# JonasFrey96/Visual-Odom-Pipeline

Hardware: NVIDIA B200
Metric: tracked_keypoints_per_sec (higher is better)
Workload: dtype u8

## Files before the change

visual-odom-pipeline_b200/csrc/klt_capi.cu:

```cuda
#include <chrono>
#include <cmath>
#include <cstdio>
#include <cstdlib>
#include <cstring>
#include <algorithm>
#include <atomic>
#include <condition_variable>
#include <thread>
#include <immintrin.h>
#include <functional>
#include <mutex>
#include <new>
#include <vector>

#include "klt_common.cuh"

using namespace klt;

struct klt_ctx {
    int device = 0;
    int sm_count = 0;
    int cc_major = 0, cc_minor = 0;
    char name[128] = {0};
    cudaStream_t stream = nullptr;
// ... 52 lines not shown
    if (guard__.err != cudaSuccess) return (klt_status)guard__.err

klt_status ensure_device_ws(klt_ctx* ctx, size_t bytes)
{
    if (bytes <= ctx->d_ws_bytes) return KLT_OK;
    ctx->reuse_key[0] = 0;
    if (ctx->d_ws) { KLT_CUDA(cudaStreamSynchronize(ctx->stream)); KLT_CUDA(cudaStreamSynchronize(ctx->stream2)); cudaFree(ctx->d_ws); ctx->d_ws = nullptr; ctx->d_ws_bytes = 0; }
    bytes = align_up(bytes + bytes / 4, 1 << 20);
    cudaError_t e = cudaMalloc(&ctx->d_ws, bytes);
    if (e != cudaSuccess) return e == cudaErrorMemoryAllocation ? KLT_ERR_OUT_OF_MEMORY : (klt_status)e;
    if (cudaMemset(ctx->d_ws, 0, bytes) != cudaSuccess || cudaDeviceSynchronize() != cudaSuccess) cudaGetLastError();
    ctx->d_ws_bytes = bytes;
    return KLT_OK;
}

klt_status ensure_host_ws(klt_ctx* ctx, size_t bytes)
{
    if (bytes <= ctx->h_ws_bytes) return KLT_OK;
    if (ctx->h_ws) { KLT_CUDA(cudaStreamSynchronize(ctx->stream)); KLT_CUDA(cudaStreamSynchronize(ctx->stream2)); cudaFreeHost(ctx->h_ws); ctx->h_ws = nullptr; ctx->h_ws_dev = nullptr; ctx->h_ws_bytes = 0; }
    bytes = align_up(bytes + bytes / 4, 1 << 16);
    cudaError_t e = cudaHostAlloc(&ctx->h_ws, bytes, cudaHostAllocMapped);
    if (e != cudaSuccess) return e == cudaErrorMemoryAllocation ? KLT_ERR_OUT_OF_MEMORY : (klt_status)e;
    void* alias = nullptr;
    ctx->h_ws_dev = (cudaHostGetDevicePointer(&alias, ctx->h_ws, 0) == cudaSuccess) ? static_cast<uint8_t*>(alias) : nullptr;
    cudaGetLastError();
    ctx->h_ws_bytes = bytes;
    return KLT_OK;
}

}

struct klt_ctx::Stager {
    static constexpr int kHelpers = 3;
    static constexpr int kParts = kHelpers + 1;
    std::thread threads[kHelpers];
    std::mutex m;
    std::condition_variable cv;
    std::atomic<unsigned> gen{0};
    std::atomic<int> done[2];
    bool stop = false;
    const uint8_t* src[2] = {nullptr, nullptr};
    uint8_t* dst[2] = {nullptr, nullptr};
    size_t bytes[2] = {0, 0};

    static void slice(size_t total, int part, size_t& off, size_t& len)
    {
        const size_t per = ((total + kParts - 1) / kParts + 63) & ~(size_t)63;
        off = std::min(total, per * (size_t)part);
        len = std::min(total - off, per);
    }
    void copy_part(int job, int part)
    {
        size_t off, len;
        slice(bytes[job], part, off, len);
        if (len) std::memcpy(dst[job] + off, src[job] + off, len);
    }
    void worker(int part)
    {
        unsigned seen = 0;
        for (;;) {
            bool got = false;
            const auto t0 = std::chrono::steady_clock::now();
            for (int spin = 0;; ++spin) {
                if (gen.load(std::memory_order_acquire) != seen) { got = true; break; }
                _mm_pause();
                if ((spin & 255) == 255 && std::chrono::steady_clock::now() - t0 > std::chrono::microseconds(200)) break;
            }
            if (!got) {
                std::unique_lock<std::mutex> lk(m);
                cv.wait(lk, [&] { return stop || gen.load(std::memory_order_acquire) != seen; });
                if (stop) return;
            }
            seen = gen.load(std::memory_order_acquire);
            if (seen == 0xffffffffu) return;
            copy_part(0, part);
            done[0].fetch_add(1, std::memory_order_release);
            copy_part(1, part);
            done[1].fetch_add(1, std::memory_order_release);
        }
    }
    bool start()
    {
        done[0].store(0); done[1].store(0);
        try {
            for (int i = 0; i < kHelpers; ++i) threads[i] = std::thread(&Stager::worker, this, i);
        } catch (...) {
            shutdown();
            return false;
        }
        return true;
    }
    void shutdown()
    {
        { std::lock_guard<std::mutex> lk(m); stop = true; gen.store(0xffffffffu, std::memory_order_release); }
        cv.notify_all();
        for (auto& t : threads) if (t.joinable()) t.join();
    }
    void post(const uint8_t* s0, uint8_t* d0, size_t b0, const uint8_t* s1, uint8_t* d1, size_t b1)
    {
        src[0] = s0; dst[0] = d0; bytes[0] = b0; src[1] = s1; dst[1] = d1; bytes[1] = b1;
        done[0].store(0, std::memory_order_relaxed); done[1].store(0, std::memory_order_relaxed);
        {
            std::lock_guard<std::mutex> lk(m);
            unsigned g = gen.load(std::memory_order_relaxed) + 1;
            if (g == 0 || g == 0xffffffffu) g = 1;
            gen.store(g, std::memory_order_release);
        }
        cv.notify_all();
    }
    void finish_job(int job)
    {
        copy_part(job, kHelpers);
        while (done[job].load(std::memory_order_acquire) < kHelpers) _mm_pause();
    }
};

namespace {

bool is_pageable(const void* p)
{
    struct Entry { uintptr_t page; bool pageable; };
    thread_local Entry cache[64] = {};
    const uintptr_t page = reinterpret_cast<uintptr_t>(p) >> 12;
    Entry& e = cache[(page ^ (page >> 6)) & 63];
    if (e.page == page && page != 0) return e.pageable;
    cudaPointerAttributes a;
    const cudaError_t err = cudaPointerGetAttributes(&a, p);
    bool pageable = true;
    if (err != cudaSuccess) cudaGetLastError();
    else pageable = (a.type == cudaMemoryTypeUnregistered);
    e.page = page; e.pageable = pageable;
    return pageable;
}

klt_status ensure_host_in(klt_ctx* ctx, size_t bytes)
{
    if (bytes <= ctx->h_in_bytes) return KLT_OK;
    if (ctx->h_in) {
        KLT_CUDA(cudaStreamSynchronize(ctx->stream));
        KLT_CUDA(cudaStreamSynchronize(ctx->stream2));
        cudaFreeHost(ctx->h_in); ctx->h_in = nullptr; ctx->h_in_bytes = 0;
    }
    bytes = align_up(bytes + bytes / 4, 1 << 16);
    cudaError_t e = cudaHostAlloc(&ctx->h_in, bytes, cudaHostAllocDefault);
    if (e != cudaSuccess) return e == cudaErrorMemoryAllocation ? KLT_ERR_OUT_OF_MEMORY : (klt_status)e;
    ctx->h_in_bytes = bytes;
    return KLT_OK;
}

}

namespace {

struct PyrReuse { const unsigned* hash_new; const unsigned* hash_old; unsigned* hash_clear; unsigned long long* skipped; unsigned mask; };

klt_status pyr_build_one_launch(klt_ctx* ctx, const uint8_t* d_img, const klt_pyr_layout* lay, uint8_t* d_pyr, int first_item,
                                int n_items, cudaStream_t stream, const PyrReuse* reuse = nullptr)
{
    const int n_steps = lay->top;
    const uint8_t* src[KLT_MAX_LEVELS];
    uint8_t* dst[KLT_MAX_LEVELS];
    int w[KLT_MAX_LEVELS], h[KLT_MAX_LEVELS];
    long long sp[KLT_MAX_LEVELS], sb[KLT_MAX_LEVELS], dp[KLT_MAX_LEVELS], db[KLT_MAX_LEVELS];
    for (int l = 0; l < n_steps; ++l) {
        const klt_level& a = lay->level[l];
        const klt_level& b = lay->level[l + 1];
        src[l] = ((l == 0) ? d_img : d_pyr + a.offset) + (int64_t)first_item * a.batch_stride;
        dst[l] = d_pyr + b.offset + (int64_t)first_item * b.batch_stride;
        w[l] = a.w; h[l] = a.h; sp[l] = a.pitch; sb[l] = a.batch_stride; dp[l] = b.pitch; db[l] = b.batch_stride;
    }
    PyrFused P;
    long long n_cnt = 0;
    klt_status s = pyr_fused_plan(P, n_steps, src, dst, w, h, sp, sb, dp, db, n_items, ctx->sm_count, &n_cnt);
    if (s != KLT_OK) return s;
    cudaStreamCaptureStatus cap = cudaStreamCaptureStatusNone;
    if (cudaStreamIsCapturing(stream, &cap) != cudaSuccess) { cudaGetLastError(); cap = cudaStreamCaptureStatusNone; }
    const bool device_gen = cap != cudaStreamCaptureStatusNone;
    const long long key[6] = {lay->level[0].w, lay->level[0].h, n_steps, n_items, lay->level[0].pitch, P.s[0].rows};
    std::lock_guard<std::mutex> guard(ctx->lk_mutex);
    klt_ctx::PyrScratch* slot = nullptr;
    for (auto& sc : ctx->pyr_scratch)
        if (sc.stream == stream && std::memcmp(sc.key, key, sizeof(key)) == 0) { slot = &sc; break; }
    const size_t words = ((size_t)(n_cnt > 0 ? n_cnt : 0) + 1) / 2 * 2 + 2;
    if (!slot) {
        if (device_gen) return KLT_ERR_UNSUPPORTED;
        if (ctx->pyr_scratch.size() >= 64) {
            KLT_CUDA(cudaDeviceSynchronize());
            for (auto& sc : ctx->pyr_scratch) cudaFree(sc.cnt);
            ctx->pyr_scratch.clear();
        }
        klt_ctx::PyrScratch fresh = {stream, nullptr, nullptr, n_cnt, 0u, {key[0], key[1], key[2], key[3], key[4], key[5]}};
        void* p = nullptr;
        cudaError_t e = cudaMalloc(&p, 2 * words * sizeof(unsigned));
        if (e != cudaSuccess) return e == cudaErrorMemoryAllocation ? KLT_ERR_OUT_OF_MEMORY : (klt_status)e;
        e = cudaMemset(p, 0, 2 * words * sizeof(unsigned));
        if (e == cudaSuccess) e = cudaDeviceSynchronize();
        if (e != cudaSuccess) { cudaFree(p); return (klt_status)e; }
        fresh.cnt = static_cast<unsigned*>(p);
        fresh.cnt_dev = fresh.cnt + words;
        try { ctx->pyr_scratch.push_back(fresh); } catch (const std::bad_alloc&) { cudaFree(p); return KLT_ERR_OUT_OF_MEMORY; }
        slot = &ctx->pyr_scratch.back();
    }
    if (device_gen) {
        P.cnt = slot->cnt_dev;
        P.gen = 0u;
        P.done = reinterpret_cast<unsigned long long*>(slot->cnt_dev + words - 2);
    } else {
        P.cnt = slot->cnt;
        P.gen = ++slot->gen;
        P.done = nullptr;
    }
    if (reuse) { P.hash_new = reuse->hash_new; P.hash_old = reuse->hash_old; P.hash_clear = reuse->hash_clear; P.skipped = reuse->skipped; P.reuse_mask = reuse->mask; }
    s = pyr_fused_launch(P, device_gen, stream);
    if (s != KLT_OK && !device_gen) --slot->gen;
    return s;
}

void make_view(const klt_pyr_layout* lay, const uint8_t* img, const uint8_t* pyr, int first_item, int item_stride, PyrView& v)
{
    v.top = lay->top;
    for (int l = 0; l <= lay->top; ++l) {
        const klt_level& s = lay->level[l];
        v.lv[l].data = ((l == 0) ? img : pyr + s.offset) + (int64_t)first_item * s.batch_stride;
        v.lv[l].batch_stride = s.batch_stride * item_stride;
        v.lv[l].pitch = (int)s.pitch;
        v.lv[l].w = s.w;
        v.lv[l].h = s.h;
        v.lv[l].aligned4 = (((uintptr_t)v.lv[l].data | (uintptr_t)s.pitch | (uintptr_t)s.batch_stride) & 3) == 0;
    }
}

klt_status check_layout(const klt_pyr_layout* lay)
{
    if (!lay || lay->top < 0 || lay->top >= KLT_MAX_LEVELS || lay->batch <= 0) return KLT_ERR_INVALID_ARG;
    for (int l = 0; l <= lay->top; ++l) {
        const klt_level& s = lay->level[l];
        if (s.w <= 0 || s.h <= 0 || s.pitch < s.w || s.pitch > 0x7fffffffLL) return KLT_ERR_INVALID_ARG;
        if (lay->batch > 1 && s.batch_stride < s.pitch * (int64_t)(s.h - 1) + s.w) return KLT_ERR_INVALID_ARG;
    }
    return KLT_OK;
}

void normalise_criteria(const klt_lk_params* p, int& max_count, double& eps2)
{
    double eps;
    if ((p->crit_type & KLT_TERM_COUNT) == 0) max_count = 30;
    else max_count = p->crit_max_count < 0 ? 0 : (p->crit_max_count > 100 ? 100 : p->crit_max_count);
    if ((p->crit_type & KLT_TERM_EPS) == 0) eps = 0.01;
    else eps = p->crit_eps < 0. ? 0. : (p->crit_eps > 10. ? 10. : p->crit_eps);
    eps2 = eps * eps;
}

void set_eps_brackets(LKLaunch& L)
{
    if (L.eps2 >= 1e-30 && L.eps2 <= 1e30) {
        L.eps2_lo = std::nextafterf((float)(L.eps2 * (1.0 - 1.0 / 1048576.0)), -1.f);
        L.eps2_hi = std::nextafterf((float)(L.eps2 * (1.0 + 1.0 / 1048576.0)), 3.0e38f);
    } else {
        L.eps2_lo = -1.f;
        L.eps2_hi = __builtin_inff();
    }
}

}

extern "C" {

int klt_version(void) { return KLT_B200_VERSION; }

const char* klt_status_string(klt_status s)
{
    switch (s) {
        case KLT_OK: return "ok";
        case KLT_ERR_INVALID_ARG: return "invalid argument (cv2 would raise an assertion error)";
        case KLT_ERR_UNSUPPORTED: return "valid for OpenCV but outside libklt_b200 limits";
        case KLT_ERR_NO_DEVICE: return "no sm_100 CUDA device available (there is no CPU fallback)";
        case KLT_ERR_OUT_OF_MEMORY: return "out of memory";
        case KLT_ERR_INTERNAL: return "internal error";
        default: return s > 0 ? cudaGetErrorString((cudaError_t)s) : "unknown status";
    }
}

klt_status klt_create(int device, klt_ctx** out)
{
    if (!out) return KLT_ERR_INVALID_ARG;
    *out = nullptr;
    int n = 0;
    if (cudaGetDeviceCount(&n) != cudaSuccess || n <= 0 || device < 0 || device >= n) {
        cudaGetLastError();
        return KLT_ERR_NO_DEVICE;
    }
    cudaDeviceProp prop;
    KLT_CUDA(cudaGetDeviceProperties(&prop, device));
    if (prop.major != 10) return KLT_ERR_NO_DEVICE;
    DeviceGuard guard(device);
    if (guard.err != cudaSuccess) return (klt_status)guard.err;
    klt_ctx* ctx = new (std::nothrow) klt_ctx();
    if (!ctx) return KLT_ERR_OUT_OF_MEMORY;
    ctx->device = device;
    ctx->sm_count = prop.multiProcessorCount;
    ctx->cc_major = prop.major;
    ctx->cc_minor = prop.minor;
    std::snprintf(ctx->name, sizeof(ctx->name), "%s", prop.name);
    cudaError_t e = cudaStreamCreateWithFlags(&ctx->stream, cudaStreamNonBlocking);
    if (e == cudaSuccess) e = cudaStreamCreateWithFlags(&ctx->stream2, cudaStreamNonBlocking);
    if (e == cudaSuccess) e = cudaEventCreateWithFlags(&ctx->ev2, cudaEventDisableTiming);
    if (e != cudaSuccess) {
        if (ctx->stream) cudaStreamDestroy(ctx->stream);
        if (ctx->stream2) cudaStreamDestroy(ctx->stream2);
        delete ctx;
        return (klt_status)e;
    }
    klt_status s = lk_init(device);
    if (s != KLT_OK) { cudaStreamDestroy(ctx->stream); cudaStreamDestroy(ctx->stream2); cudaEventDestroy(ctx->ev2); delete ctx; return s; }
    *out = ctx;
    return KLT_OK;
}

klt_status klt_destroy(klt_ctx* ctx)
{
    if (!ctx) return KLT_OK;
    DeviceGuard guard(ctx->device);
    if (ctx->stream) { cudaStreamSynchronize(ctx->stream); cudaStreamDestroy(ctx->stream); }
    if (ctx->stream2) { cudaStreamSynchronize(ctx->stream2); cudaStreamDestroy(ctx->stream2); }
    if (ctx->ev2) cudaEventDestroy(ctx->ev2);
    if (ctx->stager) { ctx->stager->shutdown(); delete ctx->stager; ctx->stager = nullptr; }
    if (ctx->d_ws) cudaFree(ctx->d_ws);
    if (ctx->h_ws) cudaFreeHost(ctx->h_ws);
    if (ctx->h_in) cudaFreeHost(ctx->h_in);
    if (ctx->d_hash) cudaFree(ctx->d_hash);
    cudaDeviceSynchronize();
    for (auto& sc : ctx->pyr_scratch) cudaFree(sc.cnt);
    for (auto& t : ctx->bilateral_tabs) cudaFree(t.d_tab);
    delete ctx;
    return KLT_OK;
}

klt_status klt_device_info(klt_ctx* ctx, int* sm_count, int* cc_major, int* cc_minor, char* name, int name_len)
{
    if (!ctx) return KLT_ERR_INVALID_ARG;
    if (sm_count) *sm_count = ctx->sm_count;
    if (cc_major) *cc_major = ctx->cc_major;
    if (cc_minor) *cc_minor = ctx->cc_minor;
    if (name && name_len > 0) std::snprintf(name, (size_t)name_len, "%s", ctx->name);
    return KLT_OK;
}

klt_status klt_host_alloc(void** ptr, int64_t bytes)
{
    if (!ptr || bytes <= 0) return KLT_ERR_INVALID_ARG;
    cudaError_t e = cudaMallocHost(ptr, (size_t)bytes);
    if (e != cudaSuccess) { *ptr = nullptr; return e == cudaErrorMemoryAllocation ? KLT_ERR_OUT_OF_MEMORY : (klt_status)e; }
    return KLT_OK;
}

klt_status klt_host_free(void* ptr)
{
    if (!ptr) return KLT_OK;
    KLT_CUDA(cudaFreeHost(ptr));
    return KLT_OK;
}

klt_status klt_pyr_plan(int w, int h, int win_w, int win_h, int max_level, int batch, klt_pyr_layout* out)
{
    if (!out || w <= 0 || h <= 0 || win_w <= 2 || win_h <= 2 || max_level < 0 || batch <= 0) return KLT_ERR_INVALID_ARG;
// ... 804 lines not shown
```

visual-odom-pipeline_b200/csrc/klt_common.cuh:

```cuda
#pragma once
#include <cuda_runtime.h>
#include <stdint.h>
#include "klt_b200.h"

#if defined(__CUDA_ARCH__) && (__CUDA_ARCH__ < 1000)
#error "libklt_b200 is written for sm_100a (B200) only"
#endif

namespace klt {

struct LevelView {
    const uint8_t* data;
    long long batch_stride;
    int pitch;
    int w, h;
    int aligned4;
};

struct PyrView {
    LevelView lv[KLT_MAX_LEVELS];
    int top;
};

__host__ __device__ __forceinline__ int reflect101(int p, int len)
{
    if ((unsigned)p < (unsigned)len) return p;
    if (len == 1) return 0;
    do {
        p = (p < 0) ? -p : 2 * len - 2 - p;
    } while ((unsigned)p >= (unsigned)len);
    return p;
}

struct PerDeviceOnce {
    bool done[64] = {};
    bool needed()
    {
        int dev = 0;
        if (cudaGetDevice(&dev) != cudaSuccess || dev < 0 || dev >= 64) return true;
        if (done[dev]) return false;
        done[dev] = true;
        return true;
    }
};

__host__ __device__ __forceinline__ unsigned fastdiv_magic(unsigned d) { return ((1u << 20) + d - 1u) / d; }
__host__ __device__ __forceinline__ unsigned fastdiv(unsigned u, unsigned magic) { return (u * magic) >> 20; }

klt_status pyr_down_launch(const uint8_t* src, int w, int h, long long spitch, long long sbatch,
                           uint8_t* dst, long long dpitch, long long dbatch, int batch, int sm_count,
                           cudaStream_t stream);

struct PyrStep {
    const uint8_t* src;
    uint8_t* dst;
    long long spitch, sbatch, dpitch, dbatch;
    int w, h, dw, dh;
    int rows, tiles_x, n8, rem_nout, strips_y;
    int cnt_off;
    long long task_begin;
};
struct PyrFused {
    PyrStep s[KLT_MAX_LEVELS - 1];
    int n_steps, batch;
    long long n_tasks;
    unsigned* cnt;
    unsigned gen;
    unsigned long long* done;
    const unsigned* hash_new;
    const unsigned* hash_old;
    unsigned* hash_clear;
    unsigned long long* skipped;
    unsigned reuse_mask;
};
klt_status pyr_fused_plan(PyrFused& P, int n_steps, const uint8_t* const* src, uint8_t* const* dst, const int* w, const int* h,
                          const long long* spitch, const long long* sbatch, const long long* dpitch, const long long* dbatch,
                          int batch, int sm_count, long long* n_counters);
klt_status pyr_fused_launch(const PyrFused& P, bool device_gen, cudaStream_t stream);

klt_status repitch_launch(const uint8_t* src, long long spitch, long long sbatch, uint8_t* dst, long long dpitch,
                          long long dbatch, int w, int h, int n_img, cudaStream_t stream, unsigned* hash = nullptr);

struct LKLaunch {
    PyrView prev, next;
    const float* prev_pts;
    float* next_pts;
    uint8_t* status;
    float* err;
    int* iters;
    int n_per_pair;
    int batch;
    int win_w, win_h;
    int max_count;
    double eps2;
    float eps2_lo, eps2_hi;
    int flags;
    float min_eig_thr;
};

klt_status lk_launch(const LKLaunch& L, int sm_count, cudaStream_t stream);
klt_status track_filter_launch(const float* p0, const float* p1, const float* p0r, long long n, float max_bidir_error,
                               int w, int h, uint8_t* keep, float* bidir, cudaStream_t stream);
klt_status lk_launch_fast(const LKLaunch& L, int sm_count, int forced_wpp, cudaStream_t stream);
klt_status lk_init(int device);

int bilateral_radius(int d, double sigma_space);
int bilateral_table_capacity();
int bilateral_tables(int d, double sigma_color, double sigma_space, float* tab, int capacity);
klt_status bilateral_launch(const uint8_t* src, int w, int h, long long spitch, long long sbatch, uint8_t* dst, long long dpitch,
                            long long dbatch, int batch, int radius, int n_taps, const float* d_tab, cudaStream_t stream);

long long corners_ws_bytes(int w, int h, int batch);
klt_status corner_min_eig_launch(const uint8_t* img, long long pitch, long long batch_stride, int w, int h, int batch,
                                 int block, float* eig, long long eig_pitch, long long eig_batch_stride,
                                 const uint8_t* mask, long long mask_pitch, long long mask_batch_stride,
                                 unsigned* max_out, void* ws, cudaStream_t stream);
klt_status corner_candidates_launch(const float* eig, long long eig_pitch, long long eig_batch_stride, int w, int h, int batch,
                                    const uint8_t* mask, long long mask_pitch, long long mask_batch_stride,
                                    const unsigned* max_in, double quality, unsigned long long* keys,
                                    long long keys_batch_stride, int capacity, unsigned* count, cudaStream_t stream);
klt_status corner_sort_launch(const unsigned long long* keys, long long keys_batch_stride, const unsigned* count, int batch,
                              unsigned* rank, unsigned long long* out, long long out_batch_stride, int out_capacity,
                              cudaStream_t stream);
klt_status corner_mask_from_points_launch(const float* pts, int n, int radius, int w, int h, uint8_t* mask, long long pitch,
                                          cudaStream_t stream);

}
```

visual-odom-pipeline_b200/csrc/klt_pyramid.cu:

```cuda
#include "klt_common.cuh"

#include <cstdlib>

namespace klt {

namespace {

constexpr int kWarpsPerBlock = 8;

__device__ __forceinline__ uint32_t prmt(uint32_t a, uint32_t b, uint32_t sel)
{
    uint32_t r;
    asm("prmt.b32 %0, %1, %2, %3;" : "=r"(r) : "r"(a), "r"(b), "r"(sel));
    return r;
}
__device__ __forceinline__ uint32_t dp4a_uu(uint32_t a, uint32_t b, uint32_t c)
{
    uint32_t d;
    asm("dp4a.u32.u32 %0, %1, %2, %3;" : "=r"(d) : "r"(a), "r"(b), "r"(c));
    return d;
}
__device__ __forceinline__ uint32_t even_bytes(uint32_t w) { return prmt(w, 0u, 0x4240u); }
__device__ __forceinline__ uint32_t odd_bytes(uint32_t w) { return prmt(w, 0u, 0x4341u); }

template <int NOUT>
struct RawRow {
    uint32_t w[NOUT / 2];
    uint32_t l, r;
};

template <int NOUT, bool ALIGNED>
__device__ __forceinline__ void load_row(const uint8_t* __restrict__ row, int cb, int w, bool fast,
                                         int lane, RawRow<NOUT>& out)
{
    constexpr int NW = NOUT / 2;
    if (ALIGNED && fast) {
        if constexpr (NOUT == 8) {
            uint4 v = __ldg(reinterpret_cast<const uint4*>(row + cb));
            out.w[0] = v.x; out.w[1] = v.y; out.w[2] = v.z; out.w[3] = v.w;
        } else {
            uint2 v = __ldg(reinterpret_cast<const uint2*>(row + cb));
            out.w[0] = v.x; out.w[1] = v.y;
        }
    } else {
#pragma unroll
        for (int i = 0; i < NW; ++i) {
            uint32_t v = 0;
#pragma unroll
            for (int j = 0; j < 4; ++j)
                v |= (uint32_t)__ldg(row + reflect101(cb + 4 * i + j, w)) << (8 * j);
            out.w[i] = v;
        }
    }
    out.l = __shfl_up_sync(0xffffffffu, out.w[NW - 1], 1);
    out.r = __shfl_down_sync(0xffffffffu, out.w[0], 1);
    if (lane == 0) {
        out.l = ((uint32_t)__ldg(row + reflect101(cb - 2, w)) << 16) |
                ((uint32_t)__ldg(row + reflect101(cb - 1, w)) << 24);
    }
    if (lane == 31) out.r = (uint32_t)__ldg(row + reflect101(cb + 2 * NOUT, w));
}

template <int NOUT>
__device__ __forceinline__ void unpack_row(const RawRow<NOUT>& raw, uint32_t (&p)[NOUT + 3])
{
    constexpr int NW = NOUT / 2;
    p[0] = even_bytes(raw.l);
    p[1] = odd_bytes(raw.l);
#pragma unroll
    for (int i = 0; i < NW; ++i) {
        p[2 + 2 * i] = even_bytes(raw.w[i]);
        p[3 + 2 * i] = odd_bytes(raw.w[i]);
    }
    p[NOUT + 2] = even_bytes(raw.r);
}

template <int NOUT, bool ALIGNED>
__global__ void __launch_bounds__(kWarpsPerBlock * 32)
pyr_down_kernel(const uint8_t* __restrict__ src, int w, int h, long long spitch, long long sbatch,
                uint8_t* __restrict__ dst, int dw, int dh, long long dpitch, long long dbatch,
                int rows_per_strip, int tiles_x, int strips_y, long long n_tasks)
{
    constexpr int NW = NOUT / 2;
    constexpr int NP = NOUT + 3;
    const int lane = threadIdx.x & 31;
    const long long task = (long long)blockIdx.x * kWarpsPerBlock + (threadIdx.x >> 5);
    if (task >= n_tasks) return;

    const int tx = (int)(task % tiles_x);
    const long long t2 = task / tiles_x;
    const int sy = (int)(t2 % strips_y);
    const int b = (int)(t2 / strips_y);

    const uint8_t* __restrict__ simg = src + (long long)b * sbatch;
    uint8_t* __restrict__ dimg = dst + (long long)b * dbatch;

    const int cb = tx * (64 * NOUT) + 2 * NOUT * lane;
    const bool fast = (cb + 2 * NOUT <= w);
    const int y0 = sy * rows_per_strip;
    const int y1 = min(y0 + rows_per_strip, dh);

    uint32_t tprev[NP], rc[NP];
    {
        RawRow<NOUT> a, bq, c;
        load_row<NOUT, ALIGNED>(simg + (long long)reflect101(2 * y0 - 2, h) * spitch, cb, w, fast, lane, a);
        load_row<NOUT, ALIGNED>(simg + (long long)reflect101(2 * y0 - 1, h) * spitch, cb, w, fast, lane, bq);
        load_row<NOUT, ALIGNED>(simg + (long long)reflect101(2 * y0, h) * spitch, cb, w, fast, lane, c);
        uint32_t pa[NP], pb[NP];
        unpack_row<NOUT>(a, pa);
        unpack_row<NOUT>(bq, pb);
        unpack_row<NOUT>(c, rc);
#pragma unroll
        for (int i = 0; i < NP; ++i) tprev[i] = pa[i] + 4u * pb[i] + rc[i];
    }

    RawRow<NOUT> nxt_o, nxt_e;
    load_row<NOUT, ALIGNED>(simg + (long long)reflect101(2 * y0 + 1, h) * spitch, cb, w, fast, lane, nxt_o);
    load_row<NOUT, ALIGNED>(simg + (long long)reflect101(2 * y0 + 2, h) * spitch, cb, w, fast, lane, nxt_e);

    const int xo = cb >> 1;
    for (int y = y0; y < y1; ++y) {
        uint32_t ro[NP], re[NP];
        unpack_row<NOUT>(nxt_o, ro);
        unpack_row<NOUT>(nxt_e, re);
        if (y + 1 < y1) {
            load_row<NOUT, ALIGNED>(simg + (long long)reflect101(2 * y + 3, h) * spitch, cb, w, fast, lane, nxt_o);
            load_row<NOUT, ALIGNED>(simg + (long long)reflect101(2 * y + 4, h) * spitch, cb, w, fast, lane, nxt_e);
        }
        uint32_t v[NP];
#pragma unroll
        for (int i = 0; i < NP; ++i) {
            uint32_t t = rc[i] + 4u * ro[i] + re[i];
            v[i] = tprev[i] + t + 4u * rc[i];
            tprev[i] = t;
            rc[i] = re[i];
        }
        uint32_t s[NW];
#pragma unroll
        for (int i = 0; i < NW; ++i) {
            const uint32_t e_m = v[2 * i], o_m = v[2 * i + 1];
            const uint32_t e_c = v[2 * i + 2], o_c = v[2 * i + 3];
            const uint32_t e_p = v[2 * i + 4];
            const uint32_t a = __funnelshift_r(e_m, e_c, 16);
            const uint32_t c = __funnelshift_r(e_c, e_p, 16);
            const uint32_t oa = __funnelshift_r(o_m, o_c, 16);
            s[i] = a + c + 6u * e_c + 4u * (oa + o_c) + 0x00800080u;
        }
        uint8_t* drow = dimg + (long long)y * dpitch + xo;
        if (ALIGNED && xo + NOUT <= dw) {
            if constexpr (NOUT == 8) {
                uint2 o;
                o.x = prmt(s[0], s[1], 0x7531u);
                o.y = prmt(s[2], s[3], 0x7531u);
                *reinterpret_cast<uint2*>(drow) = o;
// ... 161 lines not shown
        }                                                                                               \
        uint32_t wo[NW + 2], we[NW + 2];                                                                \
        KLT_LOAD_ROW(KLT_SLOT(2 * (K_) + 3), wo);                                                       \
        KLT_LOAD_ROW(KLT_SLOT(2 * (K_) + 4), we);                                                       \
        KLT_ISSUE(2 * t + 7, KLT_SLOT(2 * (K_) + 7));                                                   \
        KLT_ISSUE(2 * t + 8, KLT_SLOT(2 * (K_) + 8));                                                   \
        uint32_t p_cur[NOUT], e_nxt[NOUT], v_[NOUT];                                                    \
        KLT_HORIZ(wo, 4u, e_cur, p_cur);                                                                \
        KLT_HORIZ(we, 1u, k16, e_nxt);                                                                  \
        _Pragma("unroll") for (int i = 0; i < NOUT; ++i) {                                              \
            v_[i] = (5u * e_cur[i] + p_cur[i]) + (p_prev[i] + e_nxt[i]);                                \
            p_prev[i] = p_cur[i];                                                                       \
            e_cur[i] = e_nxt[i];                                                                        \
        }                                                                                               \
        if (full_store) {                                                                               \
             \
            if constexpr (NOUT == 8) {                                                                  \
                uint2 o;                                                                                \
                o.x = prmt(v_[1] * 65536u + v_[0], v_[3] * 65536u + v_[2], 0x7531u);                    \
                o.y = prmt(v_[5] * 65536u + v_[4], v_[7] * 65536u + v_[6], 0x7531u);                    \
                *reinterpret_cast<uint2*>(drow) = o;                                                    \
            } else {                                                                                    \
                *reinterpret_cast<uint32_t*>(drow) = prmt(v_[1] * 65536u + v_[0], v_[3] * 65536u + v_[2], 0x7531u); \
            }                                                                                           \
        } else {                                                                                        \
            _Pragma("unroll") for (int i = 0; i < NOUT; ++i)                                            \
                if (xo + i < dw) drow[i] = (uint8_t)(v_[i] >> 8);                                       \
        }                                                                                               \
        drow += dpitch;                                                                                 \
        ++t;                                                                                            \
    } while (0)

#define KLT_LOOP(FIX_)                                                                                  \
    for (int t = 0; t < n_out;) {                                                                       \
        KLT_STEP(0, FIX_);                                                                              \
        if (t >= n_out) break;                                                                          \
        KLT_STEP(1, FIX_);                                                                              \
        if (t >= n_out) break;                                                                          \
        KLT_STEP(2, FIX_);                                                                              \
        if (t >= n_out) break;                                                                          \
        KLT_STEP(3, FIX_);                                                                              \
    }
    if (fix_right) { KLT_LOOP(true) } else { KLT_LOOP(false) }
#undef KLT_LOOP
    cp_async_wait<0>();
#undef KLT_STEP
#undef KLT_SLOT
#undef KLT_ISSUE
#undef KLT_FIX_RIGHT
#undef KLT_LOAD_ROW
#undef KLT_HORIZ
}

__global__ void __launch_bounds__(kWarpsPerBlock * 32, kRingCtasPerSm)
pyr_down_ring_kernel(const uint8_t* __restrict__ src, int w, int h, long long spitch, long long sbatch,
                     uint8_t* __restrict__ dst, int dw, int dh, long long dpitch, long long dbatch,
                     int rows_per_strip, int tiles_x, int n8, int rem_nout, int strips_y, long long n_tasks)
{
    extern __shared__ __align__(128) uint8_t ring_smem[];
    const int lane = threadIdx.x & 31;
    const int warp = threadIdx.x >> 5;
    const long long task = (long long)blockIdx.x * kWarpsPerBlock + warp;
    if (task >= n_tasks) return;
    const int tx = (int)(task % tiles_x);
    const long long t2 = task / tiles_x;
    const int sy = (int)(t2 % strips_y);
    const int b = (int)(t2 / strips_y);
    const uint8_t* __restrict__ simg = src + (long long)b * sbatch;
    uint8_t* __restrict__ dimg = dst + (long long)b * dbatch;
    const uint32_t ring_s = (uint32_t)__cvta_generic_to_shared(ring_smem) + (uint32_t)(warp * RingCfg<8>::WARP_BYTES);
    const int X0 = tx * RingCfg<8>::BODY;
    const int y0 = sy * rows_per_strip;
    const int y1 = min(y0 + rows_per_strip, dh);
    if (tx < n8 || rem_nout == 8) ring_task<8>(simg, w, h, spitch, dimg, dw, dpitch, X0, y0, y1, ring_s, lane);
    else ring_task<4>(simg, w, h, spitch, dimg, dw, dpitch, X0, y0, y1, ring_s, lane);
}

int ring_rows(int dh, int tiles_x, int batch, long long resident)
{
    int rows = 2;
    double best = 1e300;
    for (int r = 2; r <= 48; ++r) {
        const int strips = (dh + r - 1) / r;
        const int rr = (dh + strips - 1) / strips;
        const long long tasks = (long long)tiles_x * strips * batch;
        const long long rounds = (tasks + resident - 1) / resident;
        const double cost = (double)rounds * (2.0 * rr + 3.0 + 6.0);
        if (cost < best) { best = cost; rows = rr; }
    }
    return rows;
}

klt_status launch_ring(const uint8_t* src, int w, int h, long long spitch, long long sbatch, uint8_t* dst,
                       int dw, int dh, long long dpitch, long long dbatch, int batch, int sm_count, cudaStream_t stream)
{
    using RC = RingCfg<8>;
    static PerDeviceOnce configured;
    const int smem = RC::WARP_BYTES * kWarpsPerBlock;
    if (configured.needed()) {
        cudaError_t e = cudaFuncSetAttribute(pyr_down_ring_kernel, cudaFuncAttributeMaxDynamicSharedMemorySize, smem);
        if (e != cudaSuccess) return (klt_status)e;
    }
    const int n8 = w / RC::BODY, rem = w - n8 * RC::BODY;
    const int rem_nout = (rem == 0) ? 0 : (rem <= RingCfg<4>::BODY ? 4 : 8);
    const int tiles_x = n8 + (rem > 0);
    const int rows = ring_rows(dh, tiles_x, batch, (long long)sm_count * kRingCtasPerSm * kWarpsPerBlock);
    const int strips_y = (dh + rows - 1) / rows;
    const long long n_tasks = (long long)tiles_x * strips_y * batch;
    const long long blocks = (n_tasks + kWarpsPerBlock - 1) / kWarpsPerBlock;
    if (blocks <= 0 || blocks > 0x7fffffffLL) return KLT_ERR_UNSUPPORTED;
    pyr_down_ring_kernel<<<(unsigned)blocks, kWarpsPerBlock * 32, smem, stream>>>(
        src, w, h, spitch, sbatch, dst, dw, dh, dpitch, dbatch, rows, tiles_x, n8, rem_nout, strips_y, n_tasks);
    cudaError_t e = cudaGetLastError();
    return e == cudaSuccess ? KLT_OK : (klt_status)e;
}

template <bool DEVGEN>
__global__ void __launch_bounds__(kWarpsPerBlock * 32, kRingCtasPerSm)
pyr_build_fused_kernel(const __grid_constant__ PyrFused P)
{
    extern __shared__ __align__(128) uint8_t ring_smem[];
    __shared__ unsigned cta_done;
    const int lane = threadIdx.x & 31;
    const int warp = threadIdx.x >> 5;
    const long long task = (long long)blockIdx.x * kWarpsPerBlock + warp;
    if constexpr (DEVGEN) {
        if (threadIdx.x == 0) cta_done = 0u;
        __syncthreads();
    }
    if (task >= P.n_tasks) return;
    int l = 0;
    while (l + 1 < P.n_steps && task >= P.s[l + 1].task_begin) ++l;
    const PyrStep& S = P.s[l];
    const long long local = task - S.task_begin;
    const int tx = (int)(local % S.tiles_x);
    const long long t2 = local / S.tiles_x;
    const int sy = (int)(t2 % S.strips_y);
    const int b = (int)(t2 / S.strips_y);
    const int y0 = sy * S.rows;
    const int y1 = min(y0 + S.rows, S.dh);
    unsigned gen = P.gen;
    if constexpr (DEVGEN) {
        if (l > 0) gen = (unsigned)(*reinterpret_cast<const volatile unsigned long long*>(P.done) / gridDim.x) + 1u;
    }
    auto sign_off = [&]() {
        if constexpr (DEVGEN) {
            if (lane == 0) {
                const long long first = (long long)blockIdx.x * kWarpsPerBlock;
                const unsigned cta_tasks = (unsigned)min((long long)kWarpsPerBlock, P.n_tasks - first);
                if (atomicAdd(&cta_done, 1u) == cta_tasks - 1u) atomicAdd(P.done, 1ull);
            }
        }
    };
    if (P.hash_new != nullptr) {
        if (task == 0 && lane == 0) { P.hash_clear[0] = 0u; P.hash_clear[1] = 0u; P.hash_clear[2] = 0u; P.hash_clear[3] = 0u; }
        if (b < 32 && ((P.reuse_mask >> b) & 1u) && P.hash_new[2 * b] == P.hash_old[2 * b] && P.hash_new[2 * b + 1] == P.hash_old[2 * b + 1]) {
            if (lane == 0) {
                if (l + 1 < P.n_steps) atomicAdd(P.cnt + S.cnt_off + (long long)b * S.strips_y + sy, 1u);
                if (l == 0 && tx == 0 && sy == 0 && P.skipped) atomicAdd(P.skipped, 1ull);
            }
            sign_off();
            return;
        }
    }
    if (l > 0) {
        const PyrStep& Q = P.s[l - 1];
        const int s_lo = max(2 * y0 - 2, 0) / Q.rows;
        const int s_hi = min(min(2 * y1, S.h - 1) / Q.rows, Q.strips_y - 1);
        const unsigned target = gen * (unsigned)Q.tiles_x;
        const volatile unsigned* c = P.cnt + Q.cnt_off + (long long)b * Q.strips_y;
        for (int k = s_lo + lane; k <= s_hi; k += 32) {
            int spins = 0;
            while ((int)(c[k] - target) < 0 && ++spins < (1 << 24)) __nanosleep(64);
        }
        __threadfence();
        __syncwarp();
    }
    const uint8_t* __restrict__ simg = S.src + (long long)b * S.sbatch;
    uint8_t* __restrict__ dimg = S.dst + (long long)b * S.dbatch;
    const uint32_t ring_s = (uint32_t)__cvta_generic_to_shared(ring_smem) + (uint32_t)(warp * RingCfg<8>::WARP_BYTES);
    const int X0 = tx * RingCfg<8>::BODY;
    if (tx < S.n8 || S.rem_nout == 8) ring_task<8>(simg, S.w, S.h, S.spitch, dimg, S.dw, S.dpitch, X0, y0, y1, ring_s, lane);
    else ring_task<4>(simg, S.w, S.h, S.spitch, dimg, S.dw, S.dpitch, X0, y0, y1, ring_s, lane);
    if (l + 1 < P.n_steps) {
        __threadfence();
        __syncwarp();
        if (lane == 0) atomicAdd(P.cnt + S.cnt_off + (long long)b * S.strips_y + sy, 1u);
    }
    sign_off();
}

template <int NOUT, bool ALIGNED>
klt_status launch_t(const uint8_t* src, int w, int h, long long spitch, long long sbatch, uint8_t* dst,
                    int dw, int dh, long long dpitch, long long dbatch, int batch, int sm_count,
                    cudaStream_t stream)
{
    const int tiles_x = (dw + 32 * NOUT - 1) / (32 * NOUT);
    int rows = 16;
    const long long want = (long long)sm_count * kWarpsPerBlock * 4;
    while (rows > 2 && (long long)tiles_x * ((dh + rows - 1) / rows) * batch < want) rows >>= 1;
    const int strips_y = (dh + rows - 1) / rows;
    const long long n_tasks = (long long)tiles_x * strips_y * batch;
    const long long blocks = (n_tasks + kWarpsPerBlock - 1) / kWarpsPerBlock;
    if (blocks <= 0 || blocks > 0x7fffffffLL) return KLT_ERR_UNSUPPORTED;
    pyr_down_kernel<NOUT, ALIGNED><<<(unsigned)blocks, kWarpsPerBlock * 32, 0, stream>>>(
        src, w, h, spitch, sbatch, dst, dw, dh, dpitch, dbatch, rows, tiles_x, strips_y, n_tasks);
    cudaError_t e = cudaGetLastError();
    return e == cudaSuccess ? KLT_OK : (klt_status)e;
}

__device__ __forceinline__ unsigned long long mix64(unsigned long long x)
{
    x ^= x >> 30; x *= 0xbf58476d1ce4e5b9ull;
    x ^= x >> 27; x *= 0x94d049bb133111ebull;
    x ^= x >> 31;
    return x;
}

template <bool HASH>
__global__ void __launch_bounds__(256)
repitch_kernel(const uint8_t* __restrict__ src, long long spitch, long long sbatch, uint8_t* __restrict__ dst,
               long long dpitch, long long dbatch, int w, int chunks, int h, unsigned* __restrict__ hash)
{
    const int t = blockIdx.x * blockDim.x + threadIdx.x;
    const int i = blockIdx.y;
    const bool live = t < chunks * h;
    unsigned long long hv = 0ull;
    if (live) {
        const int y = t / chunks, c = t - y * chunks;
        const uint8_t* s = src + (long long)i * sbatch + (long long)y * spitch + 16 * c;
        const uintptr_t a = reinterpret_cast<uintptr_t>(s);
        const uint32_t* wp = reinterpret_cast<const uint32_t*>(a & ~(uintptr_t)3);
        const int sh = (int)(a & 3) * 8;
        const uint32_t w0 = __ldg(wp), w1 = __ldg(wp + 1), w2 = __ldg(wp + 2), w3 = __ldg(wp + 3), w4 = __ldg(wp + 4);
        uint4 o;
        o.x = __funnelshift_r(w0, w1, sh);
        o.y = __funnelshift_r(w1, w2, sh);
        o.z = __funnelshift_r(w2, w3, sh);
        o.w = __funnelshift_r(w3, w4, sh);
        *reinterpret_cast<uint4*>(dst + (long long)i * dbatch + (long long)y * dpitch + 16 * c) = o;
        if constexpr (HASH) {
            const int valid = min(16, w - 16 * c);
            uint32_t q[4] = {o.x, o.y, o.z, o.w};
#pragma unroll
            for (int k = 0; k < 4; ++k) {
                const int nb = valid - 4 * k;
                q[k] = nb >= 4 ? q[k] : (nb <= 0 ? 0u : (q[k] & (0xffffffffu >> (8 * (4 - nb)))));
            }
            const unsigned long long pos = (unsigned long long)(unsigned)t + 1ull;
            hv = mix64((((unsigned long long)q[1] << 32) | q[0]) + pos * 0x9e3779b97f4a7c15ull) +
                 mix64((((unsigned long long)q[3] << 32) | q[2]) ^ (pos * 0xc2b2ae3d27d4eb4full + 0x165667b19e3779f9ull));
        }
    }
    if constexpr (HASH) {
        __shared__ unsigned s_lo[8], s_hi[8];
        const unsigned lo = __reduce_add_sync(0xffffffffu, (unsigned)(hv & 0xffffffffull));
        const unsigned hi = __reduce_add_sync(0xffffffffu, (unsigned)(hv >> 32));
        if ((threadIdx.x & 31) == 0) { s_lo[threadIdx.x >> 5] = lo; s_hi[threadIdx.x >> 5] = hi; }
        __syncthreads();
        if (threadIdx.x == 0) {
            unsigned a = 0, b = 0;
#pragma unroll
            for (int k = 0; k < 8; ++k) { a += s_lo[k]; b += s_hi[k]; }
            if (a | b) {
                atomicAdd(hash + 2 * i, a);
                atomicAdd(hash + 2 * i + 1, b);
            }
        }
    }
}

}

klt_status repitch_launch(const uint8_t* src, long long spitch, long long sbatch, uint8_t* dst, long long dpitch,
                          long long dbatch, int w, int h, int n_img, cudaStream_t stream, unsigned* hash)
{
    if (!src || !dst || w <= 0 || h <= 0 || n_img <= 0 || n_img > 65535) return KLT_ERR_INVALID_ARG;
    if ((((uintptr_t)dst | (uintptr_t)dpitch | (uintptr_t)dbatch) & 15) != 0 || dpitch < (w + 15) / 16 * 16) return KLT_ERR_INVALID_ARG;
    const int chunks = (w + 15) / 16;
    if ((long long)chunks * h > 0x7fffff00LL) return KLT_ERR_UNSUPPORTED;
    dim3 grid((unsigned)(((long long)chunks * h + 255) / 256), n_img, 1);
    if (hash) repitch_kernel<true><<<grid, 256, 0, stream>>>(src, spitch, sbatch, dst, dpitch, dbatch, w, chunks, h, hash);
    else repitch_kernel<false><<<grid, 256, 0, stream>>>(src, spitch, sbatch, dst, dpitch, dbatch, w, chunks, h, nullptr);
    cudaError_t e = cudaGetLastError();
    return e == cudaSuccess ? KLT_OK : (klt_status)e;
}

klt_status pyr_down_launch(const uint8_t* src, int w, int h, long long spitch, long long sbatch,
                           uint8_t* dst, long long dpitch, long long dbatch, int batch, int sm_count,
                           cudaStream_t stream)
{
    if (!src || !dst || w <= 0 || h <= 0 || batch <= 0 || spitch < w) return KLT_ERR_INVALID_ARG;
    const int dw = (w + 1) / 2, dh = (h + 1) / 2;
    if (dpitch < dw) return KLT_ERR_INVALID_ARG;
    const bool aligned = (((uintptr_t)src | (uintptr_t)spitch | (uintptr_t)sbatch) % 16 == 0) &&
                         (((uintptr_t)dst | (uintptr_t)dpitch | (uintptr_t)dbatch) % 8 == 0);
    const int t8 = (dw + 255) / 256 * 256, t4 = (dw + 127) / 128 * 128;
    const bool use8 = (t8 * 3 <= dw * 4) || (t8 == t4);
    static const char* force_fallback = getenv("KLT_PYR_FALLBACK");
    if (aligned && w >= 4 && h >= 3 && (long long)h * spitch < 0x7fffffffLL && !(force_fallback && force_fallback[0] == '1'))
        return launch_ring(src, w, h, spitch, sbatch, dst, dw, dh, dpitch, dbatch, batch, sm_count, stream);
    if (aligned) {
        return use8 ? launch_t<8, true>(src, w, h, spitch, sbatch, dst, dw, dh, dpitch, dbatch, batch, sm_count, stream)
                    : launch_t<4, true>(src, w, h, spitch, sbatch, dst, dw, dh, dpitch, dbatch, batch, sm_count, stream);
    }
    return launch_t<4, false>(src, w, h, spitch, sbatch, dst, dw, dh, dpitch, dbatch, batch, sm_count, stream);
}

klt_status pyr_fused_plan(PyrFused& P, int n_steps, const uint8_t* const* src, uint8_t* const* dst, const int* w, const int* h,
                          const long long* spitch, const long long* sbatch, const long long* dpitch, const long long* dbatch,
                          int batch, int sm_count, long long* n_counters)
{
    if (n_steps < 1 || n_steps > KLT_MAX_LEVELS - 1 || batch <= 0) return KLT_ERR_UNSUPPORTED;
    using RC = RingCfg<8>;
    const long long resident = (long long)sm_count * kRingCtasPerSm * kWarpsPerBlock;
    long long tasks = 0, counters = 0;
    for (int i = 0; i < n_steps; ++i) {
        PyrStep& S = P.s[i];
        const bool aligned = (((uintptr_t)src[i] | (uintptr_t)spitch[i] | (uintptr_t)sbatch[i]) % 16 == 0) &&
                             (((uintptr_t)dst[i] | (uintptr_t)dpitch[i] | (uintptr_t)dbatch[i]) % 8 == 0);
        if (!aligned || w[i] < 4 || h[i] < 3 || (long long)h[i] * spitch[i] >= 0x7fffffffLL) return KLT_ERR_UNSUPPORTED;
        S.src = src[i]; S.dst = dst[i];
        S.spitch = spitch[i]; S.sbatch = sbatch[i]; S.dpitch = dpitch[i]; S.dbatch = dbatch[i];
        S.w = w[i]; S.h = h[i]; S.dw = (w[i] + 1) / 2; S.dh = (h[i] + 1) / 2;
        S.n8 = w[i] / RC::BODY;
        const int rem = w[i] - S.n8 * RC::BODY;
        S.rem_nout = (rem == 0) ? 0 : (rem <= RingCfg<4>::BODY ? 4 : 8);
        S.tiles_x = S.n8 + (rem > 0);
        S.rows = ring_rows(S.dh, S.tiles_x, batch, resident);
        S.strips_y = (S.dh + S.rows - 1) / S.rows;
        S.task_begin = tasks;
        S.cnt_off = (int)counters;
        tasks += (long long)S.tiles_x * S.strips_y * batch;
        if (i + 1 < n_steps) counters += (long long)S.strips_y * batch;
        if (counters > 0x7fffffffLL) return KLT_ERR_UNSUPPORTED;
    }
    P.n_steps = n_steps; P.batch = batch; P.n_tasks = tasks;
    P.hash_new = nullptr; P.hash_old = nullptr; P.hash_clear = nullptr; P.skipped = nullptr; P.reuse_mask = 0u;
    P.gen = 0u; P.done = nullptr;
    *n_counters = counters;
    return KLT_OK;
}

klt_status pyr_fused_launch(const PyrFused& P, bool device_gen, cudaStream_t stream)
{
    using RC = RingCfg<8>;
    static PerDeviceOnce configured;
    const int smem = RC::WARP_BYTES * kWarpsPerBlock;
    if (configured.needed()) {
        cudaError_t e = cudaFuncSetAttribute(pyr_build_fused_kernel<false>, cudaFuncAttributeMaxDynamicSharedMemorySize, smem);
        if (e == cudaSuccess) e = cudaFuncSetAttribute(pyr_build_fused_kernel<true>, cudaFuncAttributeMaxDynamicSharedMemorySize, smem);
        if (e != cudaSuccess) return (klt_status)e;
    }
    const long long blocks = (P.n_tasks + kWarpsPerBlock - 1) / kWarpsPerBlock;
    if (blocks <= 0 || blocks > 0x7fffffffLL) return KLT_ERR_UNSUPPORTED;
    if (device_gen) pyr_build_fused_kernel<true><<<(unsigned)blocks, kWarpsPerBlock * 32, smem, stream>>>(P);
    else pyr_build_fused_kernel<false><<<(unsigned)blocks, kWarpsPerBlock * 32, smem, stream>>>(P);
    const cudaError_t e = cudaGetLastError();
    return e == cudaSuccess ? KLT_OK : (klt_status)e;
}

}
```

Before: 28.28 million.

## Add banded single-kernel pyramid build keeping intermediate levels in shared memory

Adds a new pyramid build path where each block owns a horizontal band of one image, loads the needed source rows with cp.async into shared memory, and computes all downsampled levels in shared memory, writing only owned rows to global memory. This replaces the fused ring kernel with its inter-level global counters and atomics whenever the batch and alignment fit. The cost is recomputation of overlapping halo rows between bands and occupancy limited to one large-smem block per SM. With few bands per image, some SMs may stay idle.

```diff
diff --git a/visual-odom-pipeline_b200/csrc/klt_capi.cu b/visual-odom-pipeline_b200/csrc/klt_capi.cu
--- a/visual-odom-pipeline_b200/csrc/klt_capi.cu
+++ b/visual-odom-pipeline_b200/csrc/klt_capi.cu
@@ -228,8 +228,6 @@
 
 namespace {
 
-struct PyrReuse { const unsigned* hash_new; const unsigned* hash_old; unsigned* hash_clear; unsigned long long* skipped; unsigned mask; };
-
 klt_status pyr_build_one_launch(klt_ctx* ctx, const uint8_t* d_img, const klt_pyr_layout* lay, uint8_t* d_pyr, int first_item,
                                 int n_items, cudaStream_t stream, const PyrReuse* reuse = nullptr)
 {
@@ -244,6 +242,13 @@
         src[l] = ((l == 0) ? d_img : d_pyr + a.offset) + (int64_t)first_item * a.batch_stride;
         dst[l] = d_pyr + b.offset + (int64_t)first_item * b.batch_stride;
         w[l] = a.w; h[l] = a.h; sp[l] = a.pitch; sb[l] = a.batch_stride; dp[l] = b.pitch; db[l] = b.batch_stride;
+    }
+    {
+        PyrBand B;
+        if (pyr_band_plan(B, n_steps, src, dst, w, h, sp, sb, dp, db, n_items, ctx->sm_count) == KLT_OK) {
+            if (reuse) B.reuse = *reuse;
+            return pyr_band_launch(B, stream);
+        }
     }
     PyrFused P;
     long long n_cnt = 0;
@@ -286,7 +291,7 @@
         P.gen = ++slot->gen;
         P.done = nullptr;
     }
-    if (reuse) { P.hash_new = reuse->hash_new; P.hash_old = reuse->hash_old; P.hash_clear = reuse->hash_clear; P.skipped = reuse->skipped; P.reuse_mask = reuse->mask; }
+    if (reuse) P.reuse = *reuse;
     s = pyr_fused_launch(P, device_gen, stream);
     if (s != KLT_OK && !device_gen) --slot->gen;
     return s;
diff --git a/visual-odom-pipeline_b200/csrc/klt_common.cuh b/visual-odom-pipeline_b200/csrc/klt_common.cuh
--- a/visual-odom-pipeline_b200/csrc/klt_common.cuh
+++ b/visual-odom-pipeline_b200/csrc/klt_common.cuh
@@ -51,6 +51,29 @@
                            uint8_t* dst, long long dpitch, long long dbatch, int batch, int sm_count,
                            cudaStream_t stream);
 
+struct PyrReuse {
+    const unsigned* hash_new;
+    const unsigned* hash_old;
+    unsigned* hash_clear;
+    unsigned long long* skipped;
+    unsigned mask;
+};
+
+struct PyrBand {
+    const uint8_t* src;
+    long long spitch, sbatch;
+    uint8_t* dst[KLT_MAX_LEVELS];
+    long long dpitch[KLT_MAX_LEVELS], dbatch[KLT_MAX_LEVELS];
+    int w[KLT_MAX_LEVELS], h[KLT_MAX_LEVELS];
+    int soff[KLT_MAX_LEVELS], spitch_s[KLT_MAX_LEVELS];
+    int top, batch, rows, bands, smem;
+    PyrReuse reuse;
+};
+klt_status pyr_band_plan(PyrBand& P, int n_steps, const uint8_t* const* src, uint8_t* const* dst, const int* w, const int* h,
+                         const long long* spitch, const long long* sbatch, const long long* dpitch, const long long* dbatch,
+                         int batch, int sm_count);
+klt_status pyr_band_launch(const PyrBand& P, cudaStream_t stream);
+
 struct PyrStep {
     const uint8_t* src;
     uint8_t* dst;
@@ -67,11 +90,7 @@
     unsigned* cnt;
     unsigned gen;
     unsigned long long* done;
-    const unsigned* hash_new;
-    const unsigned* hash_old;
-    unsigned* hash_clear;
-    unsigned long long* skipped;
-    unsigned reuse_mask;
+    PyrReuse reuse;
 };
 klt_status pyr_fused_plan(PyrFused& P, int n_steps, const uint8_t* const* src, uint8_t* const* dst, const int* w, const int* h,
                           const long long* spitch, const long long* sbatch, const long long* dpitch, const long long* dbatch,
diff --git a/visual-odom-pipeline_b200/csrc/klt_pyramid.cu b/visual-odom-pipeline_b200/csrc/klt_pyramid.cu
--- a/visual-odom-pipeline_b200/csrc/klt_pyramid.cu
+++ b/visual-odom-pipeline_b200/csrc/klt_pyramid.cu
@@ -1,5 +1,6 @@
 #include "klt_common.cuh"
 
+#include <algorithm>
 #include <cstdlib>
 
 namespace klt {
@@ -467,12 +468,13 @@
             }
         }
     };
-    if (P.hash_new != nullptr) {
-        if (task == 0 && lane == 0) { P.hash_clear[0] = 0u; P.hash_clear[1] = 0u; P.hash_clear[2] = 0u; P.hash_clear[3] = 0u; }
-        if (b < 32 && ((P.reuse_mask >> b) & 1u) && P.hash_new[2 * b] == P.hash_old[2 * b] && P.hash_new[2 * b + 1] == P.hash_old[2 * b + 1]) {
+    const PyrReuse& R = P.reuse;
+    if (R.hash_new != nullptr) {
+        if (task == 0 && lane == 0) { R.hash_clear[0] = 0u; R.hash_clear[1] = 0u; R.hash_clear[2] = 0u; R.hash_clear[3] = 0u; }
+        if (b < 32 && ((R.mask >> b) & 1u) && R.hash_new[2 * b] == R.hash_old[2 * b] && R.hash_new[2 * b + 1] == R.hash_old[2 * b + 1]) {
             if (lane == 0) {
                 if (l + 1 < P.n_steps) atomicAdd(P.cnt + S.cnt_off + (long long)b * S.strips_y + sy, 1u);
-                if (l == 0 && tx == 0 && sy == 0 && P.skipped) atomicAdd(P.skipped, 1ull);
+                if (l == 0 && tx == 0 && sy == 0 && R.skipped) atomicAdd(R.skipped, 1ull);
             }
             sign_off();
             return;
@@ -503,6 +505,150 @@
         if (lane == 0) atomicAdd(P.cnt + S.cnt_off + (long long)b * S.strips_y + sy, 1u);
     }
     sign_off();
+}
+
+constexpr int kBandThreads = 512;
+constexpr int kBandMaxSmem = 227 * 1024;
+#ifndef KLT_PYR_BAND_MAX_BATCH
+#define KLT_PYR_BAND_MAX_BATCH 32
+#endif
+
+__host__ __device__ __forceinline__ int band_pitch(int w) { return (w + 32 + 15) & ~15; }
+
+__device__ __forceinline__ void band_rows(const PyrBand& P, int band, int l, int& lo, int& hi)
+{
+    lo = band * P.rows;
+    hi = min(lo + P.rows, P.h[P.top]) - 1;
+    for (int k = P.top - 1; k >= l; --k) {
+        lo = max(2 * lo - 2, 0);
+        hi = min(2 * hi + 2, P.h[k] - 1);
+    }
+}
+
+__device__ __forceinline__ void sts_u32(uint32_t a, uint32_t v) { asm volatile("st.shared.u32 [%0], %1;" ::"r"(a), "r"(v) : "memory"); }
+
+__device__ __forceinline__ void band_fix_right(uint32_t row0, int pitch, int w, int n)
+{
+    for (int i = threadIdx.x; i < 2 * n; i += kBandThreads) {
+        const uint32_t a = row0 + (uint32_t)((i >> 1) * pitch + w + (i & 1));
+        sts_u8(a, lds_u8(a - 2 - 2 * (i & 1)));
+    }
+}
+
+__device__ __forceinline__ void band_horiz(const uint32_t (&W)[4], uint32_t m, const uint32_t (&init)[4], uint32_t (&out)[4])
+{
+#pragma unroll
+    for (int k = 0; k < 2; ++k) {
+        out[2 * k] = dp4a_uu(W[k], 0x04010000u * m, dp4a_uu(W[k + 1], 0x00010406u * m, init[2 * k]));
+        out[2 * k + 1] = dp4a_uu(W[k + 1], 0x04060401u * m, dp4a_uu(W[k + 2], 0x00000001u * m, init[2 * k + 1]));
+    }
+}
+
+__global__ void __launch_bounds__(kBandThreads)
+pyr_build_band_kernel(const __grid_constant__ PyrBand P)
+{
+    extern __shared__ __align__(16) uint8_t band_smem[];
+    const int band = blockIdx.x, b = blockIdx.y;
+    const PyrReuse& R = P.reuse;
+    if (R.hash_new != nullptr) {
+        if (band == 0 && b == 0 && threadIdx.x < 4) R.hash_clear[threadIdx.x] = 0u;
+        if (b < 32 && ((R.mask >> b) & 1u) && R.hash_new[2 * b] == R.hash_old[2 * b] && R.hash_new[2 * b + 1] == R.hash_old[2 * b + 1]) {
+            if (band == 0 && threadIdx.x == 0 && R.skipped) atomicAdd(R.skipped, 1ull);
+            return;
+        }
+    }
+    const uint32_t smem0 = (uint32_t)__cvta_generic_to_shared(band_smem);
+    int lo, hi;
+    band_rows(P, band, 0, lo, hi);
+    {
+        const int n = hi - lo + 1, gran = (P.w[0] + 15) >> 4;
+        const uint8_t* __restrict__ g = P.src + (long long)b * P.sbatch + (long long)lo * P.spitch;
+        const uint32_t s = smem0 + (uint32_t)(P.soff[0] + 16);
+        for (int i = threadIdx.x; i < n * gran; i += kBandThreads) {
+            const int r = i / gran, k = i - r * gran;
+            cp_async_16(s + (uint32_t)(r * P.spitch_s[0] + 16 * k), g + (long long)r * P.spitch + 16 * k);
+        }
+        cp_async_commit();
+        cp_async_wait<0>();
+        __syncthreads();
+        band_fix_right(s, P.spitch_s[0], P.w[0], n);
+        __syncthreads();
+    }
+    for (int l = 0; l < P.top; ++l) {
+        int dlo, dhi;
+        band_rows(P, band, l + 1, dlo, dhi);
+        const int sh = P.top - (l + 1);
+        const int own_lo = (band * P.rows) << sh;
+        const int own_hi = (band + 1 == (int)gridDim.x) ? P.h[l + 1] : min(((band + 1) * P.rows) << sh, P.h[l + 1]);
+        const int h = P.h[l], dw = P.w[l + 1];
+        const uint32_t sbuf = smem0 + (uint32_t)(P.soff[l] + 16);
+        const int spit = P.spitch_s[l];
+        const bool to_smem = l + 1 < P.top;
+        const uint32_t dbuf = to_smem ? smem0 + (uint32_t)(P.soff[l + 1] + 16) : 0u;
+        const int dpit = to_smem ? P.spitch_s[l + 1] : 0;
+        uint8_t* __restrict__ gdst = P.dst[l + 1] + (long long)b * P.dbatch[l + 1];
+        const long long gpitch = P.dpitch[l + 1];
+        const int G = (dw + 3) >> 2, n = dhi - dlo + 1;
+        const int C = max(1, min(n, kBandThreads / G));
+        const int len = (n + C - 1) / C;
+        for (int task = threadIdx.x; task < G * C; task += kBandThreads) {
+            const int c = task / G, g = task - c * G;
+            const int ya = dlo + c * len, yb = min(ya + len, dhi + 1);
+            if (ya >= yb) continue;
+            const int cb = 8 * g;
+            auto load = [&](int r, uint32_t (&W)[4]) {
+                const uint32_t a = sbuf + (uint32_t)((reflect101(r, h) - lo) * spit + cb);
+                const uint2 v = lds_v2(a);
+                W[0] = lds_u32(a - 4);
+                W[1] = v.x; W[2] = v.y;
+                W[3] = lds_u32(a + 8);
+                if (g == 0) W[0] = prmt(W[1], W[1], 0x1200u);
+            };
+            const uint32_t k16[4] = {16u, 16u, 16u, 16u};
+            uint32_t e_cur[4], p_prev[4];
+            {
+                uint32_t wa[4], wb[4], wc[4], e_m1[4];
+                load(2 * ya - 2, wa);
+                load(2 * ya - 1, wb);
+                load(2 * ya, wc);
+                band_horiz(wa, 1u, k16, e_m1);
+                band_horiz(wb, 4u, e_m1, p_prev);
+                band_horiz(wc, 1u, k16, e_cur);
+            }
+            const int xo = 4 * g;
+            for (int y = ya; y < yb; ++y) {
+                uint32_t wo[4], we[4], p_cur[4], e_nxt[4], v[4];
+                load(2 * y + 1, wo);
+                load(2 * y + 2, we);
+                band_horiz(wo, 4u, e_cur, p_cur);
+                band_horiz(we, 1u, k16, e_nxt);
+#pragma unroll
+                for (int i = 0; i < 4; ++i) {
+                    v[i] = (5u * e_cur[i] + p_cur[i]) + (p_prev[i] + e_nxt[i]);
+                    p_prev[i] = p_cur[i];
+                    e_cur[i] = e_nxt[i];
+                }
+                const uint32_t o = prmt(v[1] * 65536u + v[0], v[3] * 65536u + v[2], 0x7531u);
+                if (to_smem) sts_u32(dbuf + (uint32_t)((y - dlo) * dpit + xo), o);
+                if (y >= own_lo && y < own_hi) {
+                    uint8_t* __restrict__ d = gdst + (long long)y * gpitch + xo;
+                    if (xo + 4 <= dw) {
+                        *reinterpret_cast<uint32_t*>(d) = o;
+                    } else {
+#pragma unroll
+                        for (int i = 0; i < 4; ++i)
+                            if (xo + i < dw) d[i] = (uint8_t)(o >> (8 * i));
+                    }
+                }
+            }
+        }
+        lo = dlo;
+        if (to_smem) {
+            __syncthreads();
+            band_fix_right(dbuf, dpit, dw, n);
+            __syncthreads();
+        }
+    }
 }
 
 template <int NOUT, bool ALIGNED>
@@ -651,7 +797,7 @@
         if (counters > 0x7fffffffLL) return KLT_ERR_UNSUPPORTED;
     }
     P.n_steps = n_steps; P.batch = batch; P.n_tasks = tasks;
-    P.hash_new = nullptr; P.hash_old = nullptr; P.hash_clear = nullptr; P.skipped = nullptr; P.reuse_mask = 0u;
+    P.reuse = PyrReuse{nullptr, nullptr, nullptr, nullptr, 0u};
     P.gen = 0u; P.done = nullptr;
     *n_counters = counters;
     return KLT_OK;
@@ -675,4 +821,56 @@
     return e == cudaSuccess ? KLT_OK : (klt_status)e;
 }
 
-}
+klt_status pyr_band_plan(PyrBand& P, int n_steps, const uint8_t* const* src, uint8_t* const* dst, const int* w, const int* h,
+                         const long long* spitch, const long long* sbatch, const long long* dpitch, const long long* dbatch,
+                         int batch, int sm_count)
+{
+    if (n_steps < 1 || n_steps > KLT_MAX_LEVELS - 1 || batch <= 0 || batch > KLT_PYR_BAND_MAX_BATCH || batch > 65535)
+        return KLT_ERR_UNSUPPORTED;
+    if ((((uintptr_t)src[0] | (uintptr_t)spitch[0] | (uintptr_t)sbatch[0]) % 16) != 0) return KLT_ERR_UNSUPPORTED;
+    P.src = src[0]; P.spitch = spitch[0]; P.sbatch = sbatch[0];
+    P.w[0] = w[0]; P.h[0] = h[0];
+    for (int i = 0; i < n_steps; ++i) {
+        if (w[i] < 4) return KLT_ERR_UNSUPPORTED;
+        if ((((uintptr_t)dst[i] | (uintptr_t)dpitch[i] | (uintptr_t)dbatch[i]) % 4) != 0) return KLT_ERR_UNSUPPORTED;
+        P.dst[i + 1] = dst[i]; P.dpitch[i + 1] = dpitch[i]; P.dbatch[i + 1] = dbatch[i];
+        P.w[i + 1] = (w[i] + 1) / 2; P.h[i + 1] = (h[i] + 1) / 2;
+    }
+    const int ht = P.h[n_steps];
+    const int bands_max = std::max(1, sm_count / batch);
+    int n_rows[KLT_MAX_LEVELS];
+    for (int rows = (ht + bands_max - 1) / bands_max;; --rows) {
+        if (rows < 1) return KLT_ERR_UNSUPPORTED;
+        P.bands = (ht + rows - 1) / rows;
+        P.rows = (ht + P.bands - 1) / P.bands;
+        long long smem = 0;
+        for (int l = n_steps - 1, n = P.rows; l >= 0; --l) {
+            n = std::min(2 * n + 3, P.h[l]);
+            n_rows[l] = n;
+            smem += (long long)n * band_pitch(P.w[l]);
+        }
+        if (smem <= kBandMaxSmem) { P.smem = (int)smem; break; }
+    }
+    for (int l = 0, off = 0; l < n_steps; ++l) {
+        P.soff[l] = off;
+        P.spitch_s[l] = band_pitch(P.w[l]);
+        off += n_rows[l] * P.spitch_s[l];
+    }
+    P.top = n_steps; P.batch = batch;
+    P.reuse = PyrReuse{nullptr, nullptr, nullptr, nullptr, 0u};
+    return KLT_OK;
+}
+
+klt_status pyr_band_launch(const PyrBand& P, cudaStream_t stream)
+{
+    static PerDeviceOnce configured;
+    if (configured.needed()) {
+        cudaError_t e = cudaFuncSetAttribute(pyr_build_band_kernel, cudaFuncAttributeMaxDynamicSharedMemorySize, kBandMaxSmem);
+        if (e != cudaSuccess) return (klt_status)e;
+    }
+    pyr_build_band_kernel<<<dim3((unsigned)P.bands, (unsigned)P.batch), kBandThreads, P.smem, stream>>>(P);
+    const cudaError_t e = cudaGetLastError();
+    return e == cudaSuccess ? KLT_OK : (klt_status)e;
+}
+
+}
```

Result: faster. 29.86 million (median of 6 runs) (+5.6%).
